# namascar/correlation

Measured on AMD Instinct MI355X. Metric: correlation-point-iterations/sec, higher is better.
Workload: dtype f32

## Files before the change

correlation_amd/csrc/lk_kernels.hip:

```cpp
#include "lk_device.hpp"
#include "lk_launch.hpp"

#include <float.h>
#include <stdlib.h>

#include <atomic>

#include "lk_rect_walk.hpp"
#include "lk_solver_common.hpp"

namespace {

struct LevelCtx {
  gptr<uint8_t> und, def;
  gptr<f32x2> xy;
  int rx, ry, rw;
  int n;
  int urows, ucols, drows, dcols;
  float cx, cy, scaling;
};

__device__ __forceinline__ float row16_sum(float v) {
  v = dpp_add<0xB1>(v);
  v = dpp_add<0x4E>(v);
// ... 698 lines not shown
    o.und_lo = (uint32_t)ub, o.und_hi = (uint32_t)(ub >> 32), o.def_lo = (uint32_t)db, o.def_hi = (uint32_t)(db >> 32);
    o.xy_lo = (uint32_t)xb, o.xy_hi = (uint32_t)(xb >> 32);
    o.inv_rh = 1.f / (float)o.rh;
    const float4 *src = reinterpret_cast<const float4 *>(&o);
    float4 *dst = reinterpret_cast<float4 *>(ctx + row);
#pragma unroll
    for (int i = 0; i < 6; ++i)
      dst[i] = src[i];
  }
  __builtin_amdgcn_fence(__ATOMIC_RELEASE, "wavefront");
  __builtin_amdgcn_wave_barrier();
  __builtin_amdgcn_fence(__ATOMIC_ACQUIRE, "wavefront");
  int rem[4], used[4];
#pragma unroll
  for (int r = 0; r < 4; ++r) {
    rem[r] = (__builtin_amdgcn_readlane(c.n, 16 * r) + 15) >> 4;
    used[r] = 0;
  }
  const int v0 = g < N ? g : 0, v1 = (TWO && g + 16 < N) ? g + 16 : 0;
  float acc0 = 0.f, acc1 = 0.f, tot0 = 0.f, tot1 = 0.f;
  const int T = CHUNKED ? (threads < 1 ? 1 : threads) : 1;
  const int cq = c.n / T, cr = c.n - cq * T;
  int t_idx = 0, next_b = cq + (cr > 0 ? 1 : 0), kpos = 0;
  unsigned bad_sectors = 0u;
  OrdCtx e{};
  int cur = -1;
  while ((rem[0] | rem[1] | rem[2] | rem[3]) != 0) {
    int cnt[4], spare = 4;
#pragma unroll
    for (int r = 0; r < 4; ++r) {
      cnt[r] = rem[r] > 0 ? 1 : 0;
      spare -= cnt[r];
    }
    for (; spare > 0; --spare) {
      int best = -1, best_rem = 0, best_cnt = 1;
#pragma unroll
      for (int r = 0; r < 4; ++r)
        if (rem[r] > cnt[r] && (best < 0 || rem[r] * best_cnt > best_rem * cnt[r]))
          best = r, best_rem = rem[r], best_cnt = cnt[r];
      if (best < 0)
        break;
#pragma unroll
      for (int r = 0; r < 4; ++r)
        cnt[r] += best == r ? 1 : 0;
    }
    const int off1 = cnt[0], off2 = off1 + cnt[1], off3 = off2 + cnt[2], off4 = off3 + cnt[3];
    int trips = 0x7fffffff;
#pragma unroll
    for (int r = 0; r < 4; ++r)
      if (cnt[r] > 0)
        trips = min(trips, cnt[r] == 1 ? rem[r] : cnt[r] == 2 ? rem[r] >> 1 : cnt[r] == 3 ? (int)(((unsigned)rem[r] * 0xAAABu) >> 17) : rem[r] >> 2);
    const int my_sec = row >= off4 ? -1 : (row >= off1 ? 1 : 0) + (row >= off2 ? 1 : 0) + (row >= off3 ? 1 : 0);
    const int sec_off = my_sec == 1 ? off1 : my_sec == 2 ? off2 : my_sec == 3 ? off3 : 0;
    const int my_rank = row - sec_off;
    const int sec_used = my_sec == 0 ? used[0] : my_sec == 1 ? used[1] : my_sec == 2 ? used[2] : used[3];
    const int sec_cnt = my_sec == 0 ? cnt[0] : my_sec == 1 ? cnt[1] : my_sec == 2 ? cnt[2] : cnt[3];
    const int my_first = row == 0 ? 0 : row == 1 ? off1 : row == 2 ? off2 : off3;
    const int my_cnt = row == 0 ? cnt[0] : row == 1 ? cnt[1] : row == 2 ? cnt[2] : cnt[3];
    const int most = max(max(cnt[0], cnt[1]), max(cnt[2], cnt[3]));
    if (__any(my_sec >= 0 && my_sec != cur)) {
      const int want = my_sec >= 0 ? my_sec : (cur >= 0 ? cur : 0);
      const float4 *src = reinterpret_cast<const float4 *>(ctx + want);
      float4 *dst = reinterpret_cast<float4 *>(&e);
#pragma unroll
      for (int i = 0; i < 6; ++i)
        dst[i] = src[i];
      cur = want;
    }
    gptr<uint8_t> und = (gptr<uint8_t>)(uintptr_t)(((unsigned long long)e.und_hi << 32) | e.und_lo);
    gptr<uint8_t> def = (gptr<uint8_t>)(uintptr_t)(((unsigned long long)e.def_hi << 32) | e.def_lo);
    gptr<f32x2> xyl = (gptr<f32x2>)(uintptr_t)(((unsigned long long)e.xy_hi << 32) | e.xy_lo);
    const int n_mine = my_sec >= 0 ? e.n : 0;
    int k = ((sec_used + my_rank) << 4) + g;
    const int k_step = sec_cnt << 4;
    for (int trip = 0; trip < trips; ++trip, k += k_step) {
      float t[N];
#pragma unroll
      for (int v = 0; v < N; ++v)
        t[v] = 0.f;
      bool bad = false;
      if (k < n_mine) {
        f32x2 q;
        if (e.rw > 0) {
          const int rh = e.rh;
          int col = (int)((float)k * e.inv_rh);
          int rr = k - col * rh;
#pragma unroll
          for (int fix = 0; fix < 2; ++fix) {
            const int lo = rr < 0 ? 1 : 0, hi = rr >= rh ? 1 : 0;
            rr += (lo - hi) * rh;
            col += hi - lo;
          }
          q.x = (float)(e.rx + col);
          q.y = (float)(e.ry + rr);
        } else {
          q = xyl[k];
        }
        float xd, yd, dx = 0.f, dy = 0.f;
        Warp<MODEL>::apply(q.x, q.y, e.cx, e.cy, e.p, xd, yd, dx, dy);
        int uix = (int)(q.x + 0.5f), uiy = (int)(q.y + 0.5f);
        uix = min(max(uix, 0), e.ucols - 1);
        uiy = min(max(uiy, 0), e.urows - 1);
        const float und_w = (float)und[(size_t)uiy * (size_t)e.ucols + (size_t)uix];
        float W, Wx, Wy;
        if (!sample_def<INTERP>(def, e.drows, e.dcols, xd, yd, W, Wx, Wy)) {
          bad = true;
        } else {
          const float V = und_w - W;
          float H[P];
          Warp<MODEL>::jac(Wx, Wy, dx, dy, H);
          int idx = 0;
#pragma unroll
          for (int p1 = 0; p1 < P; ++p1)
#pragma unroll
            for (int p2 = p1; p2 < P; ++p2)
              t[idx++] = H[p1] * H[p2];
#pragma unroll
          for (int p1 = 0; p1 < P; ++p1)
            t[SumsT::NA + p1] = H[p1] * V;
          t[N - 1] = V * V;
        }
      }
      {
        const unsigned long long bm = __ballot(bad);
        if (bm != 0ull) {
#pragma unroll
          for (int tr = 0; tr < 4; ++tr)
            if (tr < off4 && ((bm >> (16 * tr)) & 0xffffull) != 0ull)
              bad_sectors |= 1u << ((tr >= off1 ? 1 : 0) + (tr >= off2 ? 1 : 0) + (tr >= off3 ? 1 : 0));
        }
      }
      __builtin_amdgcn_fence(__ATOMIC_RELEASE, "wavefront");
#pragma unroll
      for (int v = 0; v < N; ++v)
        tile[v * STR + lane] = t[v];
      __builtin_amdgcn_fence(__ATOMIC_RELEASE, "wavefront");
      __builtin_amdgcn_wave_barrier();
      __builtin_amdgcn_fence(__ATOMIC_ACQUIRE, "wavefront");
      for (int j = 0; j < most; ++j) {
        if (j < my_cnt) {
          const int tr = my_first + j;
          const float *r0 = tile + v0 * STR + 16 * tr, *r1 = tile + v1 * STR + 16 * tr;
#pragma unroll
          for (int j4 = 0; j4 < 4; ++j4) {
            const float4 a4 = *reinterpret_cast<const float4 *>(r0 + 4 * j4);
            float4 b4 = make_float4(0.f, 0.f, 0.f, 0.f);
            if constexpr (TWO)
              b4 = *reinterpret_cast<const float4 *>(r1 + 4 * j4);
            const float av[4] = {a4.x, a4.y, a4.z, a4.w}, bv[4] = {b4.x, b4.y, b4.z, b4.w};
#pragma unroll
            for (int jj = 0; jj < 4; ++jj) {
              if (CHUNKED && kpos + 4 * j4 + jj == next_b) {
                tot0 += acc0;
                acc0 = 0.f;
                if constexpr (TWO) {
                  tot1 += acc1;
                  acc1 = 0.f;
                }
                ++t_idx;
                next_b += cq + (t_idx < cr ? 1 : 0);
              }
              acc0 += av[jj];
              if constexpr (TWO)
                acc1 += bv[jj];
            }
          }
          kpos += 16;
        }
      }
    }
#pragma unroll
    for (int r = 0; r < 4; ++r) {
      used[r] += trips * cnt[r];
      rem[r] -= trips * cnt[r];
    }
  }
  tot0 += acc0;
  if constexpr (TWO)
    tot1 += acc1;
  __builtin_amdgcn_fence(__ATOMIC_RELEASE, "wavefront");
  float *back = tile + row * 32;
  if (g < N)
    back[g] = tot0;
  if constexpr (TWO)
    if (g + 16 < N)
      back[g + 16] = tot1;
  __builtin_amdgcn_fence(__ATOMIC_RELEASE, "wavefront");
  __builtin_amdgcn_wave_barrier();
  __builtin_amdgcn_fence(__ATOMIC_ACQUIRE, "wavefront");
#pragma unroll
  for (int v = 0; v < N; ++v)
    S.v[v] = back[v];
  __builtin_amdgcn_fence(__ATOMIC_RELEASE, "wavefront");
  return ((bad_sectors >> row) & 1u) != 0u;
}


enum : int { PH_EVAL0 = 0, PH_TENT = 1, PH_REEVAL = 2, PH_FETCH = 3, PH_EXIT = 4, PH_WAIT = 5 };
constexpr int kStaleIterations = (int)0x80000000;

struct Cold {
  float lg_p[6];
  float lambda, lg_chi, c0x, c0y;
  int iteration, reached, error, level, level_old, s, use_saved;
  uint32_t n_evals, n_sample_evals, n_point_iters;
  uint32_t n_ill;
  int sums_kept;
};
constexpr int kColdWords = sizeof(Cold) / 4;
static_assert(kColdWords % 4 == 2 && kColdWords + 7 <= kLkMidWords, "slot = 128-bit words + one 64-bit; the parked-sector record holds it");

template <bool IN_LDS, bool VEC = false> struct ColdStore {
  Cold reg;
  __device__ __forceinline__ Cold load(const uint32_t *slot) const {
    if constexpr (IN_LDS && VEC) {
      Cold k;
      uint4 *w = reinterpret_cast<uint4 *>(&k);
      const uint4 *src = reinterpret_cast<const uint4 *>(slot);
#pragma unroll
      for (int i = 0; i < kColdWords / 4; ++i)
        w[i] = src[i];
      *reinterpret_cast<uint2 *>(w + kColdWords / 4) = *reinterpret_cast<const uint2 *>(src + kColdWords / 4);
      return k;
    } else if constexpr (IN_LDS) {
      Cold k;
      uint32_t *w = reinterpret_cast<uint32_t *>(&k);
#pragma unroll
      for (int i = 0; i < kColdWords; ++i)
        w[i] = slot[i];
      return k;
    } else {
      return reg;
    }
  }
  __device__ __forceinline__ void store(uint32_t *slot, const Cold &k) {
    if constexpr (IN_LDS && VEC) {
      const uint4 *w = reinterpret_cast<const uint4 *>(&k);
      uint4 *dst = reinterpret_cast<uint4 *>(slot);
#pragma unroll
      for (int i = 0; i < kColdWords / 4; ++i)
        dst[i] = w[i];
      *reinterpret_cast<uint2 *>(dst + kColdWords / 4) = *reinterpret_cast<const uint2 *>(w + kColdWords / 4);
    } else if constexpr (IN_LDS) {
      const uint32_t *w = reinterpret_cast<const uint32_t *>(&k);
#pragma unroll
      for (int i = 0; i < kColdWords; ++i)
        slot[i] = w[i];
    } else {
      reg = k;
    }
  }
};

template <bool ON> struct HotState {
  __device__ __forceinline__ void take(const Cold &) {}
  __device__ __forceinline__ void give(Cold &) const {}
};
template <> struct HotState<true> {
  float lambda = 0.f, lg_chi = 0.f;
  int iteration = 0;
  uint32_t n_evals = 0u, n_sample_evals = 0u, n_point_iters = 0u;
  __device__ __forceinline__ void take(const Cold &k) {
    lambda = k.lambda, lg_chi = k.lg_chi, iteration = k.iteration;
    n_evals = k.n_evals, n_sample_evals = k.n_sample_evals, n_point_iters = k.n_point_iters;
  }
  __device__ __forceinline__ void give(Cold &k) const {
    k.lambda = lambda, k.lg_chi = lg_chi, k.iteration = iteration;
    k.n_evals = n_evals, k.n_sample_evals = n_sample_evals, k.n_point_iters = n_point_iters;
  }
};

#ifndef LK_MIN_WAVES
#define LK_MIN_WAVES 1
#endif
#ifndef LK_MIN_WAVES_512
#define LK_MIN_WAVES_512 1
#endif
#ifdef LK_TRACE
__device__ unsigned long long g_lk_trace[8 * 16384];
#endif
template <int MODEL, int INTERP, int GROUP, int THREADS, bool SAFE, bool REF = false, bool SEQ = false>
__global__ void __launch_bounds__(THREADS, (THREADS == 64 ? (GROUP == 16 && !SAFE && !REF ? 4 : LK_MIN_WAVES) : THREADS == 512 ? LK_MIN_WAVES_512 : 1)) lk_solve_kernel(LkSolveArgs a) {
  static_assert(!REF || (SAFE && ((THREADS == kWave && (GROUP == 16 || GROUP == kWave)) || (THREADS == 512 && GROUP == 512))), "reference-order instances");
  static_assert(!SEQ || (THREADS == kWave && GROUP >= 16 && GROUP <= kWave), "frame-pipelined instances: one wavefront per workgroup");
  if constexpr (SEQ) {
    if (a.seq_gate && __hip_atomic_load(a.seq_gate, __ATOMIC_RELAXED, __HIP_MEMORY_SCOPE_AGENT) == 0u)
      return;
  }
  constexpr int P = n_params(MODEL);
  using SumsT = Sums<P>;
  constexpr bool COLD_IN_LDS = GROUP > 1 && GROUP <= kWave;
  constexpr bool STARVED = GROUP == 1;
  constexpr bool SCATTER = GROUP == 32 && !SAFE && !REF && !SEQ && P == 6;
  const bool finisher = !REF && SAFE && GROUP == 16 && a.finisher != 0;
  constexpr bool ORD = REF;
  constexpr bool ordered_all = REF;
  const bool starved = STARVED || finisher || ordered_all;
  constexpr int RED_WORDS = GROUP > kWave ? (THREADS / kWave) * (SumsT::N + 1) + 1 : 1;
  __shared__ float lds[RED_WORDS];
  constexpr bool FLAT = REF && GROUP == 16;
  constexpr bool ORD_WG = REF && GROUP == 512;
  __shared__ __attribute__((aligned(16))) float ord_lds[FLAT ? flat_tile_floats<SumsT::N>() : ORD_WG ? wg_ord_floats<SumsT::N>() : ORD ? ord_floats<SumsT::N, (ORD && !ORD_WG) ? GROUP : 16>() : 4];
  __shared__ __attribute__((aligned(16))) OrdCtx ord_ctx[FLAT ? 4 : 1];
  constexpr bool KEEP_SUMS = GROUP == 1 || GROUP == 16;
  constexpr int kSlotWordsRaw = kColdWords + (KEEP_SUMS && COLD_IN_LDS ? SumsT::N : 0);
  constexpr int kSlotWords = GROUP == 32 ? (kSlotWordsRaw + 3) & ~3 : kSlotWordsRaw;
  __shared__ __attribute__((aligned(16))) uint32_t cold_lds[COLD_IN_LDS ? (THREADS / GROUP) * kSlotWords : 4];
  uint32_t *cold_slot = cold_lds + (COLD_IN_LDS ? ((int)threadIdx.x / GROUP) * kSlotWords : 0);
  ColdStore<COLD_IN_LDS, GROUP == 32> cold;
  HotState<SCATTER> hot;
  __shared__ float kept_lds[KEEP_SUMS && !COLD_IN_LDS ? SumsT::N * THREADS : 1];
  auto keep_sums = [&](const SumsT &v) {
    if constexpr (KEEP_SUMS && COLD_IN_LDS) {
#pragma unroll
      for (int i = 0; i < SumsT::N; ++i)
        cold_slot[kColdWords + i] = __float_as_uint(v.v[i]);
    } else if constexpr (KEEP_SUMS) {
#pragma unroll
      for (int i = 0; i < SumsT::N; ++i)
        kept_lds[i * THREADS + (int)threadIdx.x] = v.v[i];
    }
  };
  auto kept_sums = [&](SumsT &v) {
    if constexpr (KEEP_SUMS && COLD_IN_LDS) {
#pragma unroll
      for (int i = 0; i < SumsT::N; ++i)
        v.v[i] = __uint_as_float(cold_slot[kColdWords + i]);
    } else if constexpr (KEEP_SUMS) {
#pragma unroll
      for (int i = 0; i < SumsT::N; ++i)
        v.v[i] = kept_lds[i * THREADS + (int)threadIdx.x];
    }
  };

  __shared__ LkLevelView lv_lds[LK_MAX_LEVELS];
  {
    constexpr int WORDS = (int)(sizeof(LkLevelView) / 4);
    const uint32_t *src = reinterpret_cast<const uint32_t *>(a.lv);
    uint32_t *dst = reinterpret_cast<uint32_t *>(lv_lds);
    for (int i = (int)threadIdx.x; i < WORDS * (a.py_stop + 1); i += THREADS)
      dst[i] = src[i];
    __syncthreads();
  }
  float p[6];
#pragma unroll
  for (int i = 0; i < 6; ++i)
    p[i] = 0.f;
  const float min_lambda = 1e-9f, max_lambda = 1e9f;
  bool first_fetch = true;
  int phase = PH_FETCH;
  int cur_level = 0;
  LevelCtx c{};
  SumsT S;
  bool wide = false;
  int width = 16;
  int cur_frame = 0;
  uint32_t wait_spins = 0;
  constexpr bool UNIFIED = SEQ && !REF && SAFE && GROUP == 16;
  TeamCtx team;
  if constexpr (GROUP == 512) {
    if (a.team_w > 1) {
      team.w = a.team_w;
      team.rank = (int)blockIdx.x % a.team_w;
      team.slot = (int)blockIdx.x / a.team_w;
      team.partials = a.team_partials;
      team.arrivals = a.team_arrivals;
      team.n_slots = a.n_sectors;
      team.fault = a.team_fault;
      team.stride = a.team_w;
      if (a.team_min_samples > 0 && team.slot < a.n_sectors) {
        const int sector = a.order ? (int)a.order[team.slot] : team.slot;
        const LkLevelView lv0 = lv_lds[0];
        const int4 rc = lv0.rect[sector];
        const int n0 = rc.z > 0 ? rc.w : (int)(lv0.off[sector + 1] - lv0.off[sector]);
        int w = (n0 + a.team_min_samples - 1) / a.team_min_samples;
        w = w < 1 ? 1 : (w > a.team_w ? a.team_w : w);
        if (team.rank >= w)
          return;
        team.w = w;
      }
    }
  }

  auto level_count = [&](int level, int sector) -> int {
    const LkLevelView lv = lv_lds[level];
    const int4 rc = lv.rect[sector];
    return rc.z > 0 ? rc.w : (int)(lv.off[sector + 1] - lv.off[sector]);
  };

  auto hand_over = [&](const Cold &k) {
    LkHandoff h;
#pragma unroll
    for (int i = 0; i < 6; ++i)
      h.p[i] = i < P ? p[i] : 0.f;
    h.level = k.level;
    h.level_old = k.level_old;
    h.reached = k.reached;
    h.n_evals = k.n_evals;
    h.n_sample_evals = k.n_sample_evals;
    h.n_point_iters = k.n_point_iters;
    a.handoff[k.s] = h;
    phase = PH_FETCH;
  };

  auto level_context = [&](const Cold &k) {
    const LkLevelView lv = lv_lds[k.level];
    cur_level = k.level;
    const uint32_t off = lv.off[k.s];
    const int4 rc = lv.rect[k.s];
    c.rx = rc.x;
    c.ry = rc.y;
    c.rw = rc.z;
    c.n = rc.z > 0 ? rc.w : (int)(lv.off[k.s + 1] - off);
    if constexpr (SEQ) {
      c.und = (gptr<uint8_t>)a.seq_img[cur_frame].und[k.level];
      c.def = (gptr<uint8_t>)a.seq_img[cur_frame].def[k.level];
    } else {
      c.und = (gptr<uint8_t>)lv.und;
      c.def = (gptr<uint8_t>)lv.def;
    }
    const bool level_ordered = starved || (UNIFIED && c.n <= a.starved_max);
    c.xy = (gptr<f32x2>)((!level_ordered && lv.xy_eval ? lv.xy_eval : lv.xy) + off);
    c.urows = lv.urows;
    c.ucols = lv.ucols;
    c.drows = lv.drows;
    c.dcols = lv.dcols;
    c.scaling = 1.f / ((float)c.n);
    const float inv = 1.f / (float)(1 << k.level);
    c.cx = k.level == 0 ? k.c0x : k.c0x * inv;
    c.cy = k.level == 0 ? k.c0y : k.c0y * inv;
  };

  auto enter_level = [&](Cold &k) {
    translate<P>(p, k.level_old, k.level);
    k.error = LK_ERROR_NONE;
    k.lambda = 0.0001f;
    k.lg_chi = FLT_MAX;
    k.sums_kept = 0;
    level_context(k);
#pragma unroll
    for (int i = 0; i < P; ++i)
      k.lg_p[i] = p[i];
    phase = PH_EVAL0;
  };

  auto park = [&](const Cold &k, uint32_t *list, uint32_t *count) {
    uint32_t *m = a.mid_state + (size_t)k.s * kLkMidWords;
    const uint32_t *w = reinterpret_cast<const uint32_t *>(&k);
#pragma unroll
    for (int i = 0; i < kColdWords; ++i)
      m[i] = w[i];
#pragma unroll
    for (int i = 0; i < 6; ++i)
      m[kColdWords + i] = __float_as_uint(p[i]);
    m[kColdWords + 6] = (uint32_t)phase;
    const int lanes = GROUP == 32 ? (wide ? 64 : 32) : GROUP == 16 ? width : GROUP;
    if (((int)threadIdx.x & (lanes - 1)) == 0 && team.rank == 0)
      list[atomicAdd(count, 1u)] = (uint32_t)k.s;
    phase = PH_FETCH;
  };
  int steps = 0;

  auto finish_sector = [&](const Cold &k, const float (&evaluated)[6]) {
    if ((int)threadIdx.x % GROUP == 0 && team.rank == 0) {
      lk_result r;
#pragma unroll
      for (int i = 0; i < 6; ++i)
        r.resultingParameters[i] = i < P ? p[i] : 0.f;
      r.chi = k.lg_chi;
      const int4 rc0 = lv_lds[0].rect[k.s];
      r.numberOfPoints = rc0.z > 0 ? rc0.w : (int)(lv_lds[0].off[k.s + 1] - lv_lds[0].off[k.s]);
      r.iterations = (((ordered_all && a.mark_stale == 0) || a.mark_stale > 0) && k.n_evals == 1u && k.error != LK_ERROR_NONE && k.lg_chi == FLT_MAX && k.reached == 0)
                         ? kStaleIterations
                         : k.reached;
      r.errorCode = k.error;
      r.undCenterX = k.c0x;
      r.undCenterY = k.c0y;
      const size_t ridx = SEQ ? (size_t)cur_frame * (size_t)a.seq_stride + (size_t)k.s : (size_t)k.s;
      const bool state_out = !SEQ || cur_frame == a.seq_frames - 1;
      a.result[ridx] = r;
      if (a.last_p && state_out) {
#pragma unroll
        for (int i = 0; i < 6; ++i)
          a.last_p[(size_t)k.s * 6 + i] = r.resultingParameters[i];
      }
      if (a.last_eval_p && state_out) {
#pragma unroll
        for (int i = 0; i < 6; ++i)
          a.last_eval_p[(size_t)k.s * 6 + i] = a.py_start == 0 ? evaluated[i] : r.resultingParameters[i];
      }
      if (a.stats) {
        a.stats[ridx * 4 + 0] = k.n_evals;
        a.stats[ridx * 4 + 1] = k.n_sample_evals;
        a.stats[ridx * 4 + 2] = k.n_point_iters;
        a.stats[ridx * 4 + 3] = k.n_ill;
      }
      if constexpr (SEQ) {
        unsigned long long *ch = a.seq_chain + (size_t)k.s * kLkSeqChainWords + (size_t)(cur_frame & 1) * 8;
        const unsigned long long tag = (unsigned long long)(uint32_t)(cur_frame + 1) << 32;
        const bool lost = a.seq_fault != 0 && cur_frame == a.seq_fault - 1 && k.s == (a.order ? (int)a.order[0] : 0);
        if (!lost)
#pragma unroll
        for (int i = 0; i < P; ++i)
          __hip_atomic_store(ch + i, tag | (unsigned long long)__float_as_uint(r.resultingParameters[i]), __ATOMIC_RELAXED,
                             __HIP_MEMORY_SCOPE_AGENT);
      }
      if (starved && a.handoff) {
        LkHandoff h{};
        h.level = a.py_start - 1;
        a.handoff[k.s] = h;
      }
    }
    phase = PH_FETCH;
  };

#ifdef LK_TRACE
#ifndef LK_TRACE_PICK
#define LK_TRACE_PICK(G, S) ((G) > 1 && !(S))
#endif
#ifndef LK_TRACE_WHEN
#define LK_TRACE_WHEN(a) true
#endif
  const unsigned long long tr_t0 = __builtin_amdgcn_s_memrealtime();
  const unsigned long long tr_c0 = __builtin_amdgcn_s_memtime();
  unsigned long long tr_eval = 0, tr_steps = 0, tr_solve = 0, tr_fetch = 0, tr_post = 0;
  unsigned long long tr_idle = 0, tr_sleeps = 0;
#endif
  for (;;) {
    bool may_fetch = true;
    if constexpr (GROUP > 1 && GROUP < kWave) {
      if (a.align && a.persistent && !FLAT)
        may_fetch = __ballot(phase < PH_FETCH) == 0ull;
    }
    if constexpr (GROUP == 16) {
      if (width != 16 && a.align && a.persistent && may_fetch) {
        width = 16;
        cold_slot = cold_lds + ((int)threadIdx.x / GROUP) * kSlotWords;
      }
    }
#ifdef LK_TRACE_FINE
    const unsigned long long tr_f0 = __builtin_amdgcn_s_memtime();
#endif
    if (phase == PH_FETCH && may_fetch)
     for (;;) {
      int slot = 0;
      const int n_parked = (finisher || a.resume) ? (int)*(const volatile uint32_t *)a.finish_count : 0;
      if (!a.persistent) {
        const int wg_slot = ((int)blockIdx.x & 7) * a.chunk + ((int)blockIdx.x >> 3);
        slot = first_fetch ? wg_slot * (THREADS / GROUP) + (int)threadIdx.x / GROUP : a.n_sectors;
        if constexpr (FLAT) {
          if (a.rows_used > 0 && a.rows_used < 4)
            slot = (first_fetch && (int)threadIdx.x / GROUP < a.rows_used) ? wg_slot * a.rows_used + (int)threadIdx.x / GROUP : a.n_sectors;
        }
        if (GROUP == 512 && a.team_w > 1)
          slot = first_fetch ? team.slot : a.n_sectors;
        first_fetch = false;
      } else if constexpr (GROUP > kWave) {
        __syncthreads();
        if (threadIdx.x == 0)
          reinterpret_cast<int *>(lds)[RED_WORDS - 1] = (int)atomicAdd(a.queue, 1u);
        __syncthreads();
        slot = reinterpret_cast<int *>(lds)[RED_WORDS - 1];
      } else {
        if ((int)threadIdx.x % GROUP == 0)
          slot = (int)atomicAdd(a.queue, 1u);
        slot = __shfl(slot, ((int)threadIdx.x & 63) & ~(GROUP - 1), 64);
      }
      steps = 0;
      if constexpr (SEQ) {
        if (slot < a.n_sectors * a.seq_frames) {
          Cold k{};
          cur_frame = slot / a.n_sectors;
          const int pos = slot - cur_frame * a.n_sectors;
          k.s = a.order ? (int)a.order[pos] : pos;
          const float2 c0 = a.center[k.s];
          k.c0x = c0.x;
          k.c0y = c0.y;
          k.use_saved = 1;
          k.level = a.py_stop;
          k.level_old = 0;
          cold.store(cold_slot, k);
          phase = PH_WAIT;
        } else {
          phase = PH_EXIT;
        }
      } else if (finisher || a.resume) {
        if (a.resume && !finisher && (int)threadIdx.x % GROUP == 0 &&
            slot == n_parked + (int)gridDim.x * (THREADS / GROUP) - 1) {
          *a.finish_count = 0u;
          *a.queue = 0u;
        }
        if (slot < n_parked) {
          Cold k;
          const int s_idx = (int)a.finish_list[slot];
          const uint32_t *m = a.mid_state + (size_t)s_idx * kLkMidWords;
          uint32_t *w = reinterpret_cast<uint32_t *>(&k);
#pragma unroll
          for (int i = 0; i < kColdWords; ++i)
            w[i] = m[i];
#pragma unroll
          for (int i = 0; i < 6; ++i)
            p[i] = __uint_as_float(m[kColdWords + i]);
          phase = (int)m[kColdWords + 6];
          k.sums_kept = 0;
          level_context(k);
          cold.store(cold_slot, k);
          hot.take(k);
        } else {
          phase = PH_EXIT;
        }
      } else if (slot < a.n_sectors) {
        Cold k{};
        k.s = a.order ? (int)a.order[slot] : slot;
        const float2 c0 = a.center[k.s];
        k.c0x = c0.x;
        k.c0y = c0.y;
        k.use_saved = 1;
        if (!STARVED && a.handoff) {
          const LkHandoff h = a.handoff[k.s];
#pragma unroll
          for (int i = 0; i < 6; ++i)
            p[i] = i < P ? h.p[i] : 0.f;
          k.level = h.level;
          k.level_old = h.level_old;
          k.reached = h.reached;
          k.n_evals = h.n_evals;
          k.n_sample_evals = h.n_sample_evals;
          k.n_point_iters = h.n_point_iters;
        } else {
#pragma unroll
          for (int i = 0; i < 6; ++i)
            p[i] = i < P ? a.guess[(size_t)k.s * 6 + i] : 0.f;
          k.level = a.py_stop;
          k.level_old = 0;
        }
        if (k.level < a.py_start) {
          if (!a.persistent || STARVED)
            phase = PH_EXIT;
        } else if (STARVED && level_count(k.level, k.s) > a.starved_max) {
          hand_over(k);
        } else {
          enter_level(k);
          cold.store(cold_slot, k);
          hot.take(k);
        }
      } else {
        phase = PH_EXIT;
      }
      const bool all_drew_nothing = __ballot(phase != PH_FETCH) == 0ull;
      if (phase == PH_FETCH && all_drew_nothing)
        continue;
      break;
     }
#if defined(LK_TRACE_FINE) && !defined(LK_TRACE_TRANS)
    tr_fetch += __builtin_amdgcn_s_memtime() - tr_f0;
#endif
    if constexpr (SEQ) {
      if (phase == PH_WAIT) {
        Cold k = cold.load(cold_slot);
        bool ready = true;
        float g[6];
#pragma unroll
        for (int i = 0; i < 6; ++i)
          g[i] = 0.f;
        if (cur_frame == 0) {
#pragma unroll
          for (int i = 0; i < P; ++i)
            g[i] = a.guess[(size_t)k.s * 6 + i];
        } else {
          const unsigned long long *ch = a.seq_chain + (size_t)k.s * kLkSeqChainWords;
          const unsigned long long *chr = ch + (size_t)((cur_frame - 1) & 1) * 8, *chq = ch + (size_t)(cur_frame & 1) * 8;
          float r[P], q[P];
#pragma unroll
          for (int i = 0; i < P; ++i) {
            const unsigned long long x = __hip_atomic_load(chr + i, __ATOMIC_RELAXED, __HIP_MEMORY_SCOPE_AGENT);
            ready = ready && (uint32_t)(x >> 32) == (uint32_t)cur_frame;
            r[i] = __uint_as_float((uint32_t)x);
            q[i] = r[i];
          }
          if (a.seq_velocity) {
            if (cur_frame == 1) {
#pragma unroll
              for (int i = 0; i < P; ++i)
                q[i] = a.seq_prev_p[(size_t)k.s * 6 + i];
            } else {
#pragma unroll
              for (int i = 0; i < P; ++i) {
                const unsigned long long x = __hip_atomic_load(chq + i, __ATOMIC_RELAXED, __HIP_MEMORY_SCOPE_AGENT);
                ready = ready && (uint32_t)(x >> 32) == (uint32_t)(cur_frame - 1);
                q[i] = __uint_as_float((uint32_t)x);
              }
            }
          }
#pragma unroll
          for (int i = 0; i < P; ++i)
            g[i] = a.seq_velocity ? r[i] + (r[i] - q[i]) : r[i];
          if (ready && cur_frame == a.seq_frames - 1 && a.seq_prev_p_out && (int)threadIdx.x % GROUP == 0) {
#pragma unroll
            for (int i = 0; i < 6; ++i)
              a.seq_prev_p_out[(size_t)k.s * 6 + i] = i < P ? r[i] : 0.f;
          }
        }
        if (ready) {
#pragma unroll
          for (int i = 0; i < 6; ++i)
            p[i] = g[i];
          if (a.seq_guess_out && (int)threadIdx.x % GROUP == 0) {
#pragma unroll
            for (int i = 0; i < 6; ++i)
              a.seq_guess_out[((size_t)cur_frame * (size_t)a.seq_stride + (size_t)k.s) * 6 + i] = g[i];
          }
          enter_level(k);
          cold.store(cold_slot, k);
        }
      }
    }
    bool active = phase < PH_FETCH;
    if constexpr (SEQ) {
      const unsigned long long waiting = __ballot(phase == PH_WAIT);
      if (__ballot(active) == 0ull && waiting != 0ull) {
        ++wait_spins;
        const bool give_up = wait_spins > (1u << 20);
        if (give_up || (wait_spins & 255u) == 0u) {
          if (give_up || __hip_atomic_load(a.seq_flags, __ATOMIC_RELAXED, __HIP_MEMORY_SCOPE_AGENT) != 0u) {
            if (((int)threadIdx.x & 63) == 0)
              __hip_atomic_store(a.seq_flags, 1u, __ATOMIC_RELAXED, __HIP_MEMORY_SCOPE_AGENT);
            return;
          }
        }
#ifdef LK_TRACE
        ++tr_sleeps;
#endif
        __builtin_amdgcn_s_sleep(16);
        continue;
      }
      if (waiting != ~0ull)
        wait_spins = 0;
#ifdef LK_TRACE
      tr_idle += (unsigned long long)(__builtin_popcountll(~__ballot(active)) / GROUP);
#endif
    }
    if constexpr (GROUP >= kWave) {
      if (!active)
        break;
    } else {
      const unsigned long long act = __ballot(active);
      if (act == 0ull)
        break;
      if constexpr (GROUP == 32) {
        const bool lo = (uint32_t)act != 0u, hi = (uint32_t)(act >> 32) != 0u;
        if (a.solo && !wide && lo != hi && __ballot(phase == PH_EXIT) == ~act) {
          auto take = [&](auto &v) {
            const auto other = __shfl_xor(v, 32, 64);
            if (!active)
              v = other;
          };
#pragma unroll
          for (int i = 0; i < 6; ++i)
            take(p[i]);
          take(c.rx), take(c.ry), take(c.rw), take(c.n);
          take(c.urows), take(c.ucols), take(c.drows), take(c.dcols);
          take(c.scaling), take(c.cx), take(c.cy);
          auto take_ptr = [&](auto &ptr) {
            unsigned long long bits = (unsigned long long)(uintptr_t)ptr;
            uint32_t lo32 = (uint32_t)bits, hi32 = (uint32_t)(bits >> 32);
            take(lo32), take(hi32);
            ptr = (decltype(+ptr))(uintptr_t)(((unsigned long long)hi32 << 32) | lo32);
          };
          take_ptr(c.und), take_ptr(c.def), take_ptr(c.xy);
          take(phase);
          take(cur_level);
          if constexpr (SCATTER) {
            take(hot.lambda), take(hot.lg_chi), take(hot.iteration);
            take(hot.n_evals), take(hot.n_sample_evals), take(hot.n_point_iters);
          }
          if (!active)
            cold_slot = cold_lds + (((int)threadIdx.x / GROUP) ^ 1) * kSlotWords;
          active = true;
          wide = true;
        }
      }
    }
    if constexpr (GROUP == 16) {
      const unsigned long long act = __ballot(active);
      const bool idle_ok = (a.align && a.persistent) || __ballot(phase == PH_EXIT) == ~act;
      if (a.solo && width < 64 && idle_ok && !finisher && !ordered_all) {
        const unsigned rows = ((act & 0xffffull) ? 1u : 0u) | ((act & 0xffff0000ull) ? 2u : 0u) |
                              ((act & 0xffff00000000ull) ? 4u : 0u) | ((act & 0xffff000000000000ull) ? 8u : 0u);
        const unsigned sect = width == 16 ? rows : ((rows & 3u) ? 1u : 0u) | ((rows & 12u) ? 4u : 0u);
        const int n_sect = __builtin_popcount(sect);
        const int new_width = n_sect == 1 ? 64 : (n_sect == 2 && width == 16) ? 32 : width;
        if (new_width != width) {
          const int first = __builtin_ctz(sect), last = 31 - __builtin_clz(sect);
          const int lane = (int)threadIdx.x & 63;
          const int src_row = (new_width == 64 || lane < 32) ? first : last;
          const int src_lane = src_row * 16 + (lane & 15);
          auto take = [&](auto &v) { v = __shfl(v, src_lane, 64); };
#pragma unroll
          for (int i = 0; i < 6; ++i)
            take(p[i]);
          take(c.rx), take(c.ry), take(c.rw), take(c.n);
          take(c.urows), take(c.ucols), take(c.drows), take(c.dcols);
          take(c.scaling), take(c.cx), take(c.cy);
          auto take_ptr = [&](auto &ptr) {
            unsigned long long bits = (unsigned long long)(uintptr_t)ptr;
            uint32_t lo32 = (uint32_t)bits, hi32 = (uint32_t)(bits >> 32);
            take(lo32), take(hi32);
            ptr = (decltype(+ptr))(uintptr_t)(((unsigned long long)hi32 << 32) | lo32);
          };
          take_ptr(c.und), take_ptr(c.def), take_ptr(c.xy);
          take(phase);
          take(cur_level);
          int slot_idx = (int)(cold_slot - cold_lds);
          take(slot_idx);
          cold_slot = cold_lds + slot_idx;
          active = phase < PH_FETCH;
          width = new_width;
        }
      }
    }
    if constexpr (GROUP > 1 && GROUP < kWave) {
      if (a.align && !FLAT) {
        int wave_level = -1;
        for (int L = a.py_stop; L >= a.py_start && wave_level < 0; L -= a.py_step)
          if (__ballot(active && cur_level == L) != 0ull)
            wave_level = L;
        if (active && cur_level < wave_level)
          active = false;
      }
    }
    LevelCtx ce = c;
    if (!active)
      ce.n = 0;
    bool row_ordered = finisher;
    if constexpr (UNIFIED) {
      const bool ord = active && c.n <= a.starved_max;
      const bool any_plain = __ballot(active && !ord) != 0ull;
      row_ordered = active ? ord : !any_plain;
    }
#ifdef LK_TRACE
    const unsigned long long tr_e0 = __builtin_amdgcn_s_memtime();
#endif
    bool err;
    if constexpr (FLAT) {
      err = a.reference_order > 1 ? evaluate_ordered_flat<MODEL, INTERP, true>(ce, p, S, ord_lds, ord_ctx, a.reference_order)
                                  : evaluate_ordered_flat<MODEL, INTERP, false>(ce, p, S, ord_lds, ord_ctx, 1);
    } else if constexpr (ORD_WG) {
      if (team.w > 1) {
        const int T = team.w, cq = ce.n / T, cr = ce.n - cq * T;
        const int first = team.rank * cq + (team.rank < cr ? team.rank : cr), count = cq + (team.rank < cr ? 1 : 0);
        err = evaluate_ordered_wg<MODEL, INTERP, false>(ce, p, S, ord_lds, 1, first, count);
        err = team_all_to_all(S, err, lds, &team);
      } else {
        err = a.reference_order > 1 ? evaluate_ordered_wg<MODEL, INTERP, true>(ce, p, S, ord_lds, a.reference_order, 0, ce.n)
                                    : evaluate_ordered_wg<MODEL, INTERP, false>(ce, p, S, ord_lds, 1, 0, ce.n);
      }
    } else if constexpr (ORD) {
      err = a.reference_order > 1 ? evaluate_ordered<MODEL, INTERP, GROUP, true>(ce, p, S, ord_lds, a.reference_order)
                                  : evaluate_ordered<MODEL, INTERP, GROUP, false>(ce, p, S, ord_lds, 1);
    } else {
      err = evaluate<MODEL, INTERP, GROUP, THREADS, SCATTER, solve_walks_rects<MODEL, INTERP, GROUP, SAFE, REF, SEQ>()>(
          ce, p, S, lds, &team, wide, row_ordered, GROUP == 16 ? width : 0);
    }
#ifdef LK_TRACE
    tr_eval += __builtin_amdgcn_s_memtime() - tr_e0;
    ++tr_steps;
#endif
#ifdef LK_TRACE_FINE
    const unsigned long long tr_p0 = __builtin_amdgcn_s_memtime();
#endif
    if constexpr (GROUP == 512) {
      if (team.timed_out && team.w > 1) {
        if (team.rank != 0)
          return;
        team.w = 1;
        team.timed_out = false;
        phase = PH_FETCH;
        first_fetch = true;
        continue;
      }
    }
    if constexpr (SCATTER) {
      if (active && a.slot_step == 0) {
        constexpr int W_LG_P = (int)(offsetof(Cold, lg_p) / 4), W_REACHED = (int)(offsetof(Cold, reached) / 4);
        constexpr int W_USE_SAVED = (int)(offsetof(Cold, use_saved) / 4), W_N_ILL = (int)(offsetof(Cold, n_ill) / 4);
        static_assert(W_LG_P == 0, "lg_p: one 128-bit and one 64-bit access at the head of the slot");
        float evaluated[6];
#pragma unroll
        for (int i = 0; i < 6; ++i)
          evaluated[i] = p[i];
        const int evaluated_level = cur_level;
        ++hot.n_evals;
        hot.n_sample_evals += (uint32_t)c.n;
        bool level_end = false, finished = false, maxed = false, ill = false;
        if (!err) {
          const float chi = S.v[SumsT::N - 1] * c.scaling;
          const bool eval0 = phase == PH_EVAL0, tent = phase == PH_TENT;
          const float lam_down = fmaxf(hot.lambda * 0.4f, min_lambda);
          const float lam_use = tent ? lam_down : hot.lambda;
          const bool accept = eval0 || chi <= hot.lg_chi;
          const float delta_chi = __builtin_fabsf((hot.lg_chi - chi) / (fmaxf(hot.lg_chi, chi) + a.precision));
          const bool conv = tent && delta_chi < a.precision;
#ifdef LK_TRACE
          const unsigned long long tr_s0 = __builtin_amdgcn_s_memtime();
#endif
          const bool wc = damped_step_scattered(S.v[0], S.v[1], lam_use, c.scaling, p);
#ifdef LK_TRACE
          tr_solve += __builtin_amdgcn_s_memtime() - tr_s0;
#endif
          if (!wc && a.ill_list) {
            ill = true;
          } else {
            if (!wc)
              ++cold_slot[W_N_ILL];
            if (phase == PH_REEVAL) {
              phase = PH_TENT;
            } else {
              if (tent && accept) {
                *reinterpret_cast<uint4 *>(cold_slot) = make_uint4(__float_as_uint(evaluated[0]), __float_as_uint(evaluated[1]),
                                                                   __float_as_uint(evaluated[2]), __float_as_uint(evaluated[3]));
                *reinterpret_cast<uint2 *>(cold_slot + 4) = make_uint2(__float_as_uint(evaluated[4]), __float_as_uint(evaluated[5]));
              }
              hot.lambda = eval0 ? hot.lambda : accept ? lam_down : fminf(hot.lambda * 10.0f, max_lambda);
              hot.lg_chi = accept ? chi : hot.lg_chi;
              hot.iteration = eval0 ? 1 : conv ? hot.iteration : hot.iteration + 1;
              hot.n_point_iters += eval0 ? 1u : 0u;
              cold_slot[W_USE_SAVED] = accept ? 1u : 0u;
              maxed = !conv && (hot.iteration > a.max_iters || hot.lambda >= max_lambda);
              level_end = conv || maxed;
              if (!level_end) {
                cold_slot[W_REACHED] = (uint32_t)hot.iteration;
                ++hot.n_point_iters;
                phase = accept ? PH_TENT : PH_REEVAL;
                if (!accept) {
#pragma unroll
                  for (int i = 0; i < P; ++i)
                    p[i] = __uint_as_float(cold_slot[W_LG_P + i]);
                }
              }
            }
          }
        }
        if (err || ill || level_end) {
          Cold k = cold.load(cold_slot);
          hot.give(k);
          if (err) {
            k.error = LK_ERROR_INTERPOLATION_OUT_OF_IMAGE;
            if (phase == PH_EVAL0) {
              ++k.n_point_iters;
              translate<P>(p, k.level, 0);
              finished = true;
            } else {
              level_end = true;
            }
          }
          if (ill) {
            ++k.n_ill;
#pragma unroll
            for (int i = 0; i < P; ++i)
              p[i] = evaluated[i];
            --k.n_evals;
            k.n_sample_evals -= (uint32_t)c.n;
            k.sums_kept = 0;
            park(k, a.ill_list, a.ill_count);
          } else {
            if (maxed)
              k.error = LK_ERROR_CORRELATION_MAX_ITERS_REACHED;
            if (level_end) {
              k.level_old = k.level;
              k.level -= a.py_step;
              if (k.level < a.py_start) {
                translate<P>(p, k.level_old, 0);
                finished = true;
              } else {
                enter_level(k);
              }
            }
            if (finished) {
              translate<P>(evaluated, evaluated_level, 0);
              finish_sector(k, evaluated);
            } else {
              cold.store(cold_slot, k);
              hot.take(k);
            }
          }
        }
      }
    }
    if (active && (!SCATTER || a.slot_step != 0)) {
      Cold k = cold.load(cold_slot);
      float evaluated[6];
#pragma unroll
      for (int i = 0; i < 6; ++i)
        evaluated[i] = p[i];
      const int evaluated_level = k.level;
      ++k.n_evals;
      k.n_sample_evals += (uint32_t)c.n;
      bool level_end = false, iter_start = false, finished = false, handed = false;
      if (err) {
        k.error = LK_ERROR_INTERPOLATION_OUT_OF_IMAGE;
        if (phase == PH_EVAL0) {
          ++k.n_point_iters;
          translate<P>(p, k.level, 0);
          finished = true;
        } else {
          level_end = true;
        }
      } else {
        const float chi = S.v[SumsT::N - 1] * c.scaling;
        float lam_use = phase == PH_TENT ? fmaxf(k.lambda * 0.4f, min_lambda) : k.lambda;
        bool redo = false;
        if constexpr (KEEP_SUMS) {
          if (phase == PH_TENT && k.sums_kept != 0 && !(chi <= k.lg_chi)) {
            const float delta_chi = __builtin_fabsf((k.lg_chi - chi) / (fmaxf(k.lg_chi, chi) + a.precision));
            const float lambda_new = fminf(k.lambda * 10.0f, max_lambda);
            redo = !(delta_chi < a.precision) && !(k.iteration + 1 > a.max_iters || lambda_new >= max_lambda);
            if constexpr (!SAFE && !STARVED) {
              if (redo && a.ill_list) {
                float q[6];
#pragma unroll
                for (int i = 0; i < 6; ++i)
                  q[i] = p[i];
                redo = damped_step<P, false>(S, lam_use, c.scaling, q, false);
              }
            }
            if (redo) {
              k.lambda = lambda_new;
              k.use_saved = 0;
              ++k.iteration;
              k.reached = k.iteration;
              ++k.n_point_iters;
              lam_use = lambda_new;
#pragma unroll
              for (int i = 0; i < P; ++i)
                p[i] = k.lg_p[i];
            }
          }
          if (phase != PH_TENT || chi <= k.lg_chi)
            keep_sums(S);
          if (redo)
            kept_sums(S);
        }
        float tent[P];
#pragma unroll
        for (int i = 0; i < P; ++i)
          tent[i] = p[i];
#ifdef LK_TRACE
        const unsigned long long tr_s0 = __builtin_amdgcn_s_memtime();
#endif
        const bool step_starved = starved || (UNIFIED && row_ordered);
        bool wc;
        if constexpr (SCATTER)
          wc = damped_step_scattered(S.v[0], S.v[1], lam_use, c.scaling, p);
        else
          wc = damped_step<P, SAFE || STARVED>(S, lam_use, c.scaling, p, step_starved, nullptr, SAFE && GROUP >= 16 && GROUP <= kWave);
#ifdef LK_TRACE
        tr_solve += __builtin_amdgcn_s_memtime() - tr_s0;
#endif
        if (!wc && !step_starved)
          ++k.n_ill;
        if constexpr (SEQ && !SAFE) {
          if (!wc && (int)threadIdx.x % GROUP == 0)
            __hip_atomic_store(a.seq_flags + 1, 1u, __ATOMIC_RELAXED, __HIP_MEMORY_SCOPE_AGENT);
        }
        bool ill_parked = false;
        if constexpr (!SAFE && !STARVED) {
          if (!wc && a.ill_list) {
#pragma unroll
            for (int i = 0; i < P; ++i)
              p[i] = tent[i];
            if (redo) {
              phase = PH_REEVAL;
            } else {
              --k.n_evals;
              k.n_sample_evals -= (uint32_t)c.n;
            }
            k.sums_kept = 0;
            park(k, a.ill_list, a.ill_count);
            ill_parked = true;
          }
        }
        if (ill_parked) {
        } else if (redo) {
          phase = PH_TENT;
        } else if (phase == PH_EVAL0) {
          ++k.n_point_iters;
          k.lg_chi = chi;
          k.use_saved = 1;
          k.iteration = 1;
          iter_start = true;
          if constexpr (KEEP_SUMS) {
            k.sums_kept = a.keep_sums;
          }
        } else if (phase == PH_REEVAL) {
          phase = PH_TENT;
          if constexpr (KEEP_SUMS) {
            k.sums_kept = a.keep_sums;
          }
        } else {
          const float delta_chi =
              __builtin_fabsf((k.lg_chi - chi) / (fmaxf(k.lg_chi, chi) + a.precision));
          if (chi <= k.lg_chi) {
            k.lg_chi = chi;
            k.lambda = fmaxf(k.lambda * 0.4f, min_lambda);
#pragma unroll
            for (int i = 0; i < P; ++i)
              k.lg_p[i] = tent[i];
            k.use_saved = 1;
            if constexpr (KEEP_SUMS) {
              k.sums_kept = a.keep_sums;
            }
          } else {
            k.lambda = fminf(k.lambda * 10.0f, max_lambda);
            k.use_saved = 0;
          }
          if (delta_chi < a.precision) {
            level_end = true;
          } else {
            ++k.iteration;
            iter_start = true;
          }
        }
      }
#ifdef LK_TRACE_TRANS
      const unsigned long long tr_x0 = __builtin_amdgcn_s_memtime();
#endif
      if (iter_start) {
        if (k.iteration > a.max_iters || k.lambda >= max_lambda) {
          k.error = LK_ERROR_CORRELATION_MAX_ITERS_REACHED;
          level_end = true;
        } else {
          k.reached = k.iteration;
          ++k.n_point_iters;
          if (k.use_saved) {
            phase = PH_TENT;
          } else {
#pragma unroll
            for (int i = 0; i < P; ++i)
              p[i] = k.lg_p[i];
            phase = PH_REEVAL;
          }
        }
      }
      if (level_end) {
        k.level_old = k.level;
        k.level -= a.py_step;
        if (k.level < a.py_start) {
          translate<P>(p, k.level_old, 0);
          finished = true;
        } else if (starved && !ordered_all && level_count(k.level, k.s) > a.starved_max) {
          handed = true;
        } else {
          enter_level(k);
        }
      }
      if (finished) {
        translate<P>(evaluated, evaluated_level, 0);
        finish_sector(k, evaluated);
      }
      else if (handed)
        hand_over(k);
      else if (STARVED && a.eval_cap > 0 && ++steps >= a.eval_cap)
        park(k, a.finish_list, a.finish_count);
      else
        cold.store(cold_slot, k);
#ifdef LK_TRACE_TRANS
      tr_fetch += __builtin_amdgcn_s_memtime() - tr_x0;
#endif
    }
#ifdef LK_TRACE_FINE
    tr_post += __builtin_amdgcn_s_memtime() - tr_p0;
#endif
  }
#ifdef LK_TRACE
  if constexpr (LK_TRACE_PICK(GROUP, SAFE)) {
    if (((int)threadIdx.x & 63) == 0 && blockIdx.x < 16384u && LK_TRACE_WHEN(a)) {
      unsigned long long *w = g_lk_trace + 8 * ((size_t)blockIdx.x);
      unsigned hw, xcc;
      asm volatile("s_getreg_b32 %0, hwreg(HW_REG_HW_ID)" : "=s"(hw));
      asm volatile("s_getreg_b32 %0, hwreg(HW_REG_XCC_ID)" : "=s"(xcc));
      w[0] = tr_t0;
      w[1] = __builtin_amdgcn_s_memrealtime();
      w[2] = tr_eval;
      w[3] = tr_steps | ((unsigned long long)gridDim.x << 32);
#ifdef LK_TRACE_FINE
      w[4] = tr_fetch;
      w[5] = tr_post;
#else
      w[4] = SEQ ? tr_idle : hw;
      w[5] = SEQ ? tr_sleeps : xcc;
#endif
      w[6] = __builtin_amdgcn_s_memtime() - tr_c0;
      w[7] = tr_solve;
    }
  }
#endif
}

template <int MODEL, int INTERP, int GROUP>
__global__ void __launch_bounds__(256) lk_eval_kernel(LkEvalArgs a) {
  constexpr int P = n_params(MODEL);
  using SumsT = Sums<P>;
  __shared__ float lds[4 * (SumsT::N + 1)];
  constexpr int OG = GROUP == 16 ? 16 : kWave;
  __shared__ __attribute__((aligned(16))) float ord_lds[OG == 16 ? flat_tile_floats<SumsT::N>() : ord_floats<SumsT::N, OG>()];
  __shared__ __attribute__((aligned(16))) OrdCtx ord_ctx[4];
  if (a.ref_threads > 0 && (int)threadIdx.x >= kWave)
    return;
  const LkLevelView lv = a.lv[a.level];
  const uint32_t off = lv.off[a.sector];
  const float2 c0 = a.center[a.sector];
  const float inv = 1.f / (float)(1 << a.level);
  LevelCtx c{};
  const int4 rc = lv.rect[a.sector];
  c.rx = rc.x;
  c.ry = rc.y;
  c.rw = rc.z;
  c.n = rc.z > 0 ? rc.w : (int)(lv.off[a.sector + 1] - off);
  if (GROUP < kWave && (int)threadIdx.x >= GROUP)
    c.n = 0;
  c.und = (gptr<uint8_t>)lv.und;
  c.def = (gptr<uint8_t>)lv.def;
  c.xy = (gptr<f32x2>)(lv.xy + off);
  c.urows = lv.urows;
  c.ucols = lv.ucols;
  c.drows = lv.drows;
  c.dcols = lv.dcols;
  c.cx = a.level == 0 ? c0.x : c0.x * inv;
  c.cy = a.level == 0 ? c0.y : c0.y * inv;
  float p[6];
#pragma unroll
  for (int i = 0; i < 6; ++i)
    p[i] = a.p[i];
  SumsT S;
  bool err;
  if (a.ref_threads > 0) {
    if constexpr (OG == 16) {
      if ((int)threadIdx.x >= 16)
        c.n = 0;
      err = a.ref_threads > 1 ? evaluate_ordered_flat<MODEL, INTERP, true>(c, p, S, ord_lds, ord_ctx, a.ref_threads)
                              : evaluate_ordered_flat<MODEL, INTERP, false>(c, p, S, ord_lds, ord_ctx, 1);
    } else {
      err = a.ref_threads > 1 ? evaluate_ordered<MODEL, INTERP, OG, true>(c, p, S, ord_lds, a.ref_threads)
                              : evaluate_ordered<MODEL, INTERP, OG, false>(c, p, S, ord_lds, 1);
    }
  } else {
    err = evaluate<MODEL, INTERP, GROUP, 256, false, eval_walks_rects<MODEL, INTERP, GROUP>()>(c, p, S, lds);
  }
  if (threadIdx.x == 0) {
    for (int i = 0; i < 44; ++i)
      a.out[i] = 0.f;
    int idx = 0;
    for (int p1 = 0; p1 < P; ++p1)
      for (int p2 = p1; p2 < P; ++p2)
        a.out[p1 * 6 + p2] = S.v[idx++];
    for (int p1 = 0; p1 < P; ++p1)
      a.out[36 + p1] = S.v[SumsT::NA + p1];
    a.out[42] = S.v[SumsT::N - 1];
    a.out[43] = err ? 1.f : 0.f;
  }
}

template <int INTERP>
__global__ void lk_sample_kernel(const uint8_t *def, int rows, int cols, const float2 *pts, int n,
                                 float4 *out) {
  int k = (int)(blockIdx.x * blockDim.x + threadIdx.x);
  if (k >= n)
    return;
  float W = 0.f, Wx = 0.f, Wy = 0.f;
  bool ok = sample_def<INTERP>((gptr<uint8_t>)def, rows, cols, pts[k].x, pts[k].y, W, Wx, Wy);
  out[k] = ok ? make_float4(W, Wx, Wy, 0.f) : make_float4(0.f, 0.f, 0.f, 1.f);
}

template <int P> __global__ void lk_solve_only_kernel(const float *in, float *dp_out) {
  Sums<P> S;
  int idx = 0;
  for (int p1 = 0; p1 < P; ++p1)
    for (int p2 = p1; p2 < P; ++p2)
      S.v[idx++] = in[p1 * 6 + p2];
  for (int p1 = 0; p1 < P; ++p1)
    S.v[Sums<P>::NA + p1] = in[36 + p1];
  S.v[Sums<P>::N - 1] = 0.f;
  float p[6] = {0, 0, 0, 0, 0, 0}, dp[6] = {0, 0, 0, 0, 0, 0};
  damped_step<P, true>(S, in[42], in[43], p, in[44] != 0.f, dp, in[44] == 2.f);
  if (threadIdx.x == 0 && blockIdx.x == 0)
    for (int i = 0; i < 6; ++i)
      dp_out[i] = i < P ? dp[i] : 0.f;
}

__global__ void __launch_bounds__(kWave) lk_step_compare_kernel(const float *in, float *out, int n) {
  const int l = (int)threadIdx.x;
  const int b0 = l & 1, b1 = (l >> 1) & 1, b2 = (l >> 2) & 1, b3 = (l >> 3) & 1;
  const int mine = ((b0 ^ b2) << 4) | ((b1 ^ b2) << 3) | ((b2 ^ b3) << 2) | (b3 << 1);
  for (int i = (int)blockIdx.x; i < n; i += (int)gridDim.x) {
    const float *q = in + (size_t)i * 40;
    Sums<6> S;
#pragma unroll
    for (int k = 0; k < 28; ++k)
      S.v[k] = q[k];
    const float lambda = q[28], scaling = q[29];
    float pr[6], ps[6], xr[6], xs[6];
#pragma unroll
    for (int k = 0; k < 6; ++k)
      pr[k] = ps[k] = q[30 + k];
    const bool fr = damped_step<6, false>(S, lambda, scaling, pr, false, xr);
    const bool fs = damped_step_scattered(q[mine], q[mine + 1], lambda, scaling, ps, xs);
    bool same = __builtin_amdgcn_readfirstlane((int)fs) == (int)fs;
#pragma unroll
    for (int k = 0; k < 6; ++k)
      same = same && __builtin_amdgcn_readfirstlane((int)__float_as_uint(xs[k])) == (int)__float_as_uint(xs[k]) &&
             __builtin_amdgcn_readfirstlane((int)__float_as_uint(ps[k])) == (int)__float_as_uint(ps[k]);
    const bool all_same = __ballot(same) == ~0ull;
    if (l == 0) {
      float *o = out + (size_t)i * 32;
#pragma unroll
      for (int k = 0; k < 6; ++k) {
        o[k] = xr[k];
        o[6 + k] = pr[k];
        o[16 + k] = xs[k];
        o[22 + k] = ps[k];
      }
      o[12] = fr ? 1.f : 0.f;
      o[28] = fs ? 1.f : 0.f;
      o[13] = o[14] = o[15] = o[30] = o[31] = 0.f;
      o[29] = all_same ? 1.f : 0.f;
    }
// ... 1526 lines not shown
```

Before: 491.2 million.

## Keep accepted sums for group-32 scatter path to skip rejected re-evaluations

Extends the keep-sums mechanism to GROUP==32 kernels, including the scattered register-form solver. When a tentative step is rejected, it reuses the sums saved at the last accepted point to solve the retry step immediately, instead of spending a separate re-evaluation pass over the samples. This adds LDS storage per lane and a sums_kept flag in the cold slot, plus extra bookkeeping for ill-conditioned cases, at some risk of subtle state mismatches.

```diff
diff --git a/correlation_amd/csrc/lk_kernels.hip b/correlation_amd/csrc/lk_kernels.hip
--- a/correlation_amd/csrc/lk_kernels.hip
+++ b/correlation_amd/csrc/lk_kernels.hip
@@ -1024,16 +1024,21 @@
   constexpr bool ORD_WG = REF && GROUP == 512;
   __shared__ __attribute__((aligned(16))) float ord_lds[FLAT ? flat_tile_floats<SumsT::N>() : ORD_WG ? wg_ord_floats<SumsT::N>() : ORD ? ord_floats<SumsT::N, (ORD && !ORD_WG) ? GROUP : 16>() : 4];
   __shared__ __attribute__((aligned(16))) OrdCtx ord_ctx[FLAT ? 4 : 1];
-  constexpr bool KEEP_SUMS = GROUP == 1 || GROUP == 16;
-  constexpr int kSlotWordsRaw = kColdWords + (KEEP_SUMS && COLD_IN_LDS ? SumsT::N : 0);
+  constexpr bool KEEP_SUMS = GROUP == 1 || GROUP == 16 || (GROUP == 32 && !SEQ);
+  constexpr int kSlotWordsRaw = kColdWords + (KEEP_SUMS && COLD_IN_LDS && !SCATTER ? SumsT::N : 0);
   constexpr int kSlotWords = GROUP == 32 ? (kSlotWordsRaw + 3) & ~3 : kSlotWordsRaw;
   __shared__ __attribute__((aligned(16))) uint32_t cold_lds[COLD_IN_LDS ? (THREADS / GROUP) * kSlotWords : 4];
   uint32_t *cold_slot = cold_lds + (COLD_IN_LDS ? ((int)threadIdx.x / GROUP) * kSlotWords : 0);
   ColdStore<COLD_IN_LDS, GROUP == 32> cold;
   HotState<SCATTER> hot;
   __shared__ float kept_lds[KEEP_SUMS && !COLD_IN_LDS ? SumsT::N * THREADS : 1];
+  static_assert(!SCATTER || KEEP_SUMS, "the register form of the step keeps its sums unconditionally");
+  __shared__ float2 kept_lane[SCATTER ? THREADS : 1];
+  [[maybe_unused]] constexpr int W_SUMS_KEPT = (int)(offsetof(Cold, sums_kept) / 4);
   auto keep_sums = [&](const SumsT &v) {
-    if constexpr (KEEP_SUMS && COLD_IN_LDS) {
+    if constexpr (SCATTER) {
+      kept_lane[(int)threadIdx.x] = make_float2(v.v[0], v.v[1]);
+    } else if constexpr (KEEP_SUMS && COLD_IN_LDS) {
 #pragma unroll
       for (int i = 0; i < SumsT::N; ++i)
         cold_slot[kColdWords + i] = __float_as_uint(v.v[i]);
@@ -1044,7 +1049,11 @@
     }
   };
   auto kept_sums = [&](SumsT &v) {
-    if constexpr (KEEP_SUMS && COLD_IN_LDS) {
+    if constexpr (SCATTER) {
+      const float2 t = kept_lane[(int)threadIdx.x];
+      v.v[0] = t.x;
+      v.v[1] = t.y;
+    } else if constexpr (KEEP_SUMS && COLD_IN_LDS) {
 #pragma unroll
       for (int i = 0; i < SumsT::N; ++i)
         v.v[i] = __uint_as_float(cold_slot[kColdWords + i]);
@@ -1498,6 +1507,8 @@
           }
           if (!active)
             cold_slot = cold_lds + (((int)threadIdx.x / GROUP) ^ 1) * kSlotWords;
+          if constexpr (KEEP_SUMS)
+            cold_slot[W_SUMS_KEPT] = 0u;
           active = true;
           wide = true;
         }
@@ -1623,26 +1634,63 @@
           const bool accept = eval0 || chi <= hot.lg_chi;
           const float delta_chi = __builtin_fabsf((hot.lg_chi - chi) / (fmaxf(hot.lg_chi, chi) + a.precision));
           const bool conv = tent && delta_chi < a.precision;
+          float s0 = S.v[0], s1 = S.v[1], lam = lam_use;
+          if (!tent || accept)
+            kept_lane[(int)threadIdx.x] = make_float2(s0, s1);
+          if (tent && !conv && chi > hot.lg_chi && cold_slot[W_SUMS_KEPT] != 0u) {
+            const float lambda_new = fminf(hot.lambda * 10.0f, max_lambda);
+            bool redo = !(hot.iteration + 1 > a.max_iters || lambda_new >= max_lambda);
+            if (redo && a.ill_list) {
+              float q[6];
+#pragma unroll
+              for (int i = 0; i < 6; ++i)
+                q[i] = p[i];
+              redo = damped_step_scattered(s0, s1, lam, c.scaling, q);
+            }
+            if (redo) {
+              hot.lambda = lambda_new;
+              ++hot.iteration;
+              ++hot.n_point_iters;
+              cold_slot[W_USE_SAVED] = 0u;
+              cold_slot[W_REACHED] = (uint32_t)hot.iteration;
+#pragma unroll
+              for (int i = 0; i < P; ++i)
+                p[i] = __uint_as_float(cold_slot[W_LG_P + i]);
+              const float2 t = kept_lane[(int)threadIdx.x];
+              s0 = t.x, s1 = t.y, lam = lambda_new;
+              phase = PH_REEVAL;
+            }
+          }
 #ifdef LK_TRACE
           const unsigned long long tr_s0 = __builtin_amdgcn_s_memtime();
 #endif
-          const bool wc = damped_step_scattered(S.v[0], S.v[1], lam_use, c.scaling, p);
+          const bool wc = damped_step_scattered(s0, s1, lam, c.scaling, p);
 #ifdef LK_TRACE
           tr_solve += __builtin_amdgcn_s_memtime() - tr_s0;
 #endif
           if (!wc && a.ill_list) {
             ill = true;
+            if (tent && phase == PH_REEVAL) {
+              ++hot.n_evals;
+              hot.n_sample_evals += (uint32_t)c.n;
+#pragma unroll
+              for (int i = 0; i < P; ++i)
+                evaluated[i] = __uint_as_float(cold_slot[W_LG_P + i]);
+            }
           } else {
             if (!wc)
               ++cold_slot[W_N_ILL];
             if (phase == PH_REEVAL) {
               phase = PH_TENT;
+              cold_slot[W_SUMS_KEPT] = (uint32_t)a.keep_sums;
             } else {
               if (tent && accept) {
                 *reinterpret_cast<uint4 *>(cold_slot) = make_uint4(__float_as_uint(evaluated[0]), __float_as_uint(evaluated[1]),
                                                                    __float_as_uint(evaluated[2]), __float_as_uint(evaluated[3]));
                 *reinterpret_cast<uint2 *>(cold_slot + 4) = make_uint2(__float_as_uint(evaluated[4]), __float_as_uint(evaluated[5]));
               }
+              if (accept)
+                cold_slot[W_SUMS_KEPT] = (uint32_t)a.keep_sums;
               hot.lambda = eval0 ? hot.lambda : accept ? lam_down : fminf(hot.lambda * 10.0f, max_lambda);
               hot.lg_chi = accept ? chi : hot.lg_chi;
               hot.iteration = eval0 ? 1 : conv ? hot.iteration : hot.iteration + 1;
@@ -1733,7 +1781,7 @@
         float lam_use = phase == PH_TENT ? fmaxf(k.lambda * 0.4f, min_lambda) : k.lambda;
         bool redo = false;
         if constexpr (KEEP_SUMS) {
-          if (phase == PH_TENT && k.sums_kept != 0 && !(chi <= k.lg_chi)) {
+          if (phase == PH_TENT && k.sums_kept != 0 && (GROUP == 32 ? chi > k.lg_chi : !(chi <= k.lg_chi))) {
             const float delta_chi = __builtin_fabsf((k.lg_chi - chi) / (fmaxf(k.lg_chi, chi) + a.precision));
             const float lambda_new = fminf(k.lambda * 10.0f, max_lambda);
             redo = !(delta_chi < a.precision) && !(k.iteration + 1 > a.max_iters || lambda_new >= max_lambda);
@@ -1743,7 +1791,10 @@
 #pragma unroll
                 for (int i = 0; i < 6; ++i)
                   q[i] = p[i];
-                redo = damped_step<P, false>(S, lam_use, c.scaling, q, false);
+                if constexpr (SCATTER)
+                  redo = damped_step_scattered(S.v[0], S.v[1], lam_use, c.scaling, q);
+                else
+                  redo = damped_step<P, false>(S, lam_use, c.scaling, q, false);
               }
             }
             if (redo) {
```

Result: faster. 497.8 million (median of 5 runs) (+1.3%).
